# nico-bohlinger/RL-X

Hardware: AMD Instinct MI355X
Metric: env-steps/sec (whole node) PPO 4096 envs at 1/2/4/8 MI355X (higher is better)
Workload: dtype f32

## Files before the change

### include/rlx_hip.h

```cpp
#ifndef RLX_HIP_H
#define RLX_HIP_H

#include <stdint.h>

#ifdef __cplusplus
extern "C" {
#endif

#define RLX_OK 0
#define RLX_EINVAL (-1)
#define RLX_EHIP (-2)
#define RLX_ENOMEM (-3)
#define RLX_EUNSUP (-4)

#define RLX_ACT_TANH 0
#define RLX_ACT_ELU 1
#define RLX_ACT_RELU 2
#define RLX_ACT_NONE 3
#define RLX_ACT_SILU 4

#define RLX_THREEFRY_LEGACY 0
#define RLX_THREEFRY_PARTITIONABLE 1

typedef struct rlx_ctx rlx_ctx;
// ... 31 lines not shown
const char* rlx_prof_kernel_name(int k);
int rlx_prof_begin(rlx_ctx* ctx);
int rlx_prof_end(rlx_ctx* ctx, double* ms_out, double* flops_out, double* bytes_out, int64_t* count_out);
typedef struct rlx_prof_row {
  int32_t kernel;
  int32_t engine;
  int32_t N, K;
  int64_t M;
  int64_t launches, timed;
  double ms, flops, bytes;
} rlx_prof_row;
int rlx_prof_rows(rlx_ctx* ctx, rlx_prof_row* rows, int capacity, int* n_out);
int rlx_prof_union_ms(rlx_ctx* ctx, double* out);

int rlx_dbg_set_option(rlx_ctx* ctx, const char* name, int value);
int rlx_dbg_get_counter(rlx_ctx* ctx, const char* name, int64_t* out);

int rlx_dbg_set_sac_noise(rlx_ctx* ctx, const float* eps_next, const float* eps_cur);

int rlx_dbg_set_stamps(rlx_ctx* ctx, void* stamps);

int rlx_dbg_gemm_f32(rlx_ctx* ctx, int mode, const float* A, const float* B, float* C, float* aux, int64_t M, int N,
                     int K, int act, void* stream);

int rlx_dbg_l1_f32(rlx_ctx* ctx, int bwd, const float* X, const float* W, const float* b, const float* g,
                   const float* be, float* H, float* ln_partials, int64_t M, int O, int Hd, int act, int ln, int grid,
                   void* stream);

int rlx_threefry_split_host(const uint32_t key_in[2], uint32_t* keys_out , int num, int scheme);
int rlx_random_bits_u32(rlx_ctx*, const uint32_t key[2], uint32_t* out, int64_t n, int scheme, void* stream);
int rlx_normal_f32(rlx_ctx*, const uint32_t key[2], float* out, int64_t n, int scheme, void* stream);
int rlx_permutation_i32(rlx_ctx*, uint32_t key_io[2], int32_t* out, int E, int64_t B, int scheme, void* stream);

int rlx_env_reset_f32(rlx_ctx*, uint32_t seed, int env_id_offset, int N, int obs_dim, int horizon,
                      float* obs , int32_t* ep_step , float* ep_ret ,
                      float* last_ret , float* last_len , void* stream);
int rlx_env_step_f32(rlx_ctx*, uint32_t seed, int env_id_offset, uint32_t t, int N, int obs_dim, int act_dim,
                     int horizon, float p_term, float reward_noise,
                     const float* action , float* obs ,
                     float* final_obs ,
                     float* reward , float* terminated , float* truncated ,
                     int32_t* ep_step, float* ep_ret, float* last_ret, float* last_len,
                     float* episode_stats ,
                     void* stream);
int rlx_env_step_copy_f32(rlx_ctx*, uint32_t seed, int env_id_offset, uint32_t t, int N, int obs_dim, int act_dim,
                          int horizon, float p_term, float reward_noise, const float* action, float* obs, float* final_obs,
// ... 328 lines not shown
```

### rl-x_amd/csrc/common.h

```cpp
#pragma once
#include <hip/hip_runtime.h>
#include <hip/hip_ext.h>
#include <stdint.h>
#include <cstring>
#include <cmath>
#include <string>
#include <vector>
#include <functional>
#include "../../include/rlx_hip.h"

namespace rlx {

void set_error(const std::string& msg);

#define RLX_HIP_TRY(expr)                                                                      \
  do {                                                                                         \
    hipError_t e_ = (expr);                                                                    \
    if (e_ != hipSuccess) {                                                                    \
      ::rlx::set_error(std::string(#expr) + " failed: " + hipGetErrorString(e_) + " (" __FILE__ \
                       ":" + std::to_string(__LINE__) + ")");                                  \
      return RLX_EHIP;                                                                         \
    }                                                                                          \
  } while (0)

// ... 61 lines not shown
  int opt_flip = 0;
  hipStream_t side = nullptr;
  hipEvent_t ev_fork = nullptr, ev_join = nullptr;
  hipEvent_t ev_rows[2] = {nullptr, nullptr};
  hipEvent_t ev_cdone[2] = {nullptr, nullptr};
  const float* dbg_sac_eps[2] = {nullptr, nullptr};
  bool l1fwd_mfma = true;
  bool pipeline_updates = true;
  bool pf_valid = false;
  uint32_t pf_key_in[2] = {0, 0}, pf_key_out[2] = {0, 0};
  int pf_E = 0, pf_scheme = 0;
  int64_t pf_B = 0;
  hipEvent_t pf_done = nullptr;
  hipEvent_t ev_perm_free = nullptr;
  bool perm_free_recorded = false;
  bool two_streams = true;
  const uint32_t* l1_xmax = nullptr;
  const uint32_t* xmax_slot[2] = {nullptr, nullptr};
  int lf_idle_cus = 0;
  bool dw_recompute = false;
  float* l12_stats = nullptr;
  bool l12_ran = false;
  bool dw_merge = true;
  void* dbg_stamps = nullptr;
  bool fwd2h = true;
  int gather_group_rows = 524288;
  bool gather_records = true;
  bool l12_fused = true;
  int ppo_tail = -1;
  int ppo_twin = -1;
  bool fused_recurrent_act = true;
  int num_cus = 256;
  void* defer = nullptr;
  bool prof_on = false;
  int prof_sample = 1;
  hipEvent_t prof_ref = nullptr;
  double prof_union_ms = 0.0;
  std::vector<rlx::ProfRec> prof_recs;
  std::vector<rlx::ProfRow> prof_rows;
  std::vector<hipEvent_t> prof_pool;
  bool gemm_bx = true;
  float bx_gscale = 1.f;
  bool adam_emit = true;
  bool bx_keep[3] = {false, false, false};
  struct RoImages { bool valid = false; const float* params[2] = {nullptr, nullptr}; const void* img[2][3] = {}; int nt[2][3] = {}; } ro_img;
  int bx_force_mi = 0;
// ... 362 lines not shown
```

### rl-x_amd/csrc/core.hip

```cpp
#include "common.h"
#include <algorithm>
#include <cstdio>
#include <cstdlib>
#include <utility>

namespace rlx {

static thread_local std::string g_last_error;

void set_error(const std::string& msg) { g_last_error = msg; }

void* scratch(rlx_ctx* ctx, ScratchSlot s, size_t bytes) {
  Scratch& sl = ctx->slots[ctx->bank][s];
  if (sl.bytes >= bytes && sl.ptr) return sl.ptr;
  if (sl.ptr) {
    if (hipDeviceSynchronize() != hipSuccess) { set_error("hipDeviceSynchronize failed in scratch()"); return nullptr; }
    (void)hipFree(sl.ptr);
    sl.ptr = nullptr;
    sl.bytes = 0;
  }
  size_t want = ((bytes > (size_t(1) << 20) ? bytes + bytes / 8 : bytes) + 255) & ~size_t(255);
  void* p = nullptr;
  hipError_t e = hipMalloc(&p, want);
  if (e != hipSuccess) {
// ... 178 lines not shown
    rows[i] = rlx_prof_row{q.kid, q.engine, q.N, q.K, q.M, q.launches, q.timed, q.ms, q.flops, q.bytes};
  }
  return RLX_OK;
}

int rlx_prof_union_ms(rlx_ctx* ctx, double* out) {
  RLX_REQUIRE(ctx && out, RLX_EINVAL, "rlx_prof_union_ms: NULL pointer");
  *out = ctx->prof_union_ms;
  return RLX_OK;
}

int rlx_dbg_set_option(rlx_ctx* ctx, const char* name, int value) {
  RLX_REQUIRE(ctx && name, RLX_EINVAL, "rlx_dbg_set_option: NULL");
  if (std::string(name) == "sac_twin") { ctx->sac_twin = value; return RLX_OK; }
  if (std::string(name) == "disable_l1fused") { ctx->disable_l1fused = value != 0; return RLX_OK; }
  if (std::string(name) == "l1fwd_mfma") { ctx->l1fwd_mfma = value != 0; return RLX_OK; }
  if (std::string(name) == "pipeline_updates") { ctx->pipeline_updates = value != 0; return RLX_OK; }
  if (std::string(name) == "two_streams") { ctx->two_streams = value != 0; return RLX_OK; }
  if (std::string(name) == "ppo_twin") { ctx->ppo_twin = value; return RLX_OK; }
  if (std::string(name) == "ro_exit") { ctx->ro_exit = value; return RLX_OK; }
  if (std::string(name) == "lf_idle_cus") { ctx->lf_idle_cus = value < 0 ? 0 : value; return RLX_OK; }
  if (std::string(name) == "dw_recompute") { ctx->dw_recompute = value != 0; return RLX_OK; }
  if (std::string(name) == "dw_merge") { ctx->dw_merge = value != 0; return RLX_OK; }
  if (std::string(name) == "fwd2h") { ctx->fwd2h = value != 0; return RLX_OK; }
  if (std::string(name) == "l12_fused") { ctx->l12_fused = value != 0; return RLX_OK; }
  if (std::string(name) == "gather_group_rows") { ctx->gather_group_rows = value; return RLX_OK; }
  if (std::string(name) == "gather_records") { ctx->gather_records = value != 0; return RLX_OK; }
  if (std::string(name) == "ppo_tail") { ctx->ppo_tail = value < 0 ? -1 : (value > 2 ? 2 : value); return RLX_OK; }
  if (std::string(name) == "bx_force_mi") { ctx->bx_force_mi = value; return RLX_OK; }
  if (std::string(name) == "adam_emit") { ctx->adam_emit = value != 0; return RLX_OK; }
  if (std::string(name) == "bx_debug") { ctx->bx_debug = value; return RLX_OK; }
  if (std::string(name) == "bx_gscale_log2") { ctx->bx_gscale = ldexpf(1.f, value < 0 ? 0 : (value > 40 ? 40 : value)); return RLX_OK; }
  if (std::string(name) == "gemm_bx") { ctx->gemm_bx = value != 0; return RLX_OK; }
  if (std::string(name) == "prof_sample") { ctx->prof_sample = value < 1 ? 1 : value; return RLX_OK; }
  if (std::string(name) == "fused_recurrent_act") { ctx->fused_recurrent_act = value != 0; return RLX_OK; }
  RLX_REQUIRE(false, RLX_EINVAL, "rlx_dbg_set_option: unknown option");
}

int rlx_dbg_get_counter(rlx_ctx* ctx, const char* name, int64_t* out) {
  RLX_REQUIRE(ctx && name && out, RLX_EINVAL, "rlx_dbg_get_counter: NULL");
  int bank = 0, slot = 0;
  if (sscanf(name, "scratch_ptr:%d:%d", &bank, &slot) == 2 && bank >= 0 && bank < 3 && slot >= 0 && slot < rlx::SL_COUNT) {
    *out = (int64_t)reinterpret_cast<uintptr_t>(ctx->slots[bank][slot].ptr);
    return RLX_OK;
  }
  if (sscanf(name, "scratch_bytes:%d:%d", &bank, &slot) == 2 && bank >= 0 && bank < 3 && slot >= 0 && slot < rlx::SL_COUNT) {
    *out = (int64_t)ctx->slots[bank][slot].bytes;
    return RLX_OK;
  }
  if (std::string(name) == "allreduce_calls") { *out = ctx->ar_calls; return RLX_OK; }
  if (std::string(name) == "bx_window_fallbacks") { *out = ctx->bx_window_fallbacks; return RLX_OK; }
  if (std::string(name) == "gemm_bx") { *out = ctx->gemm_bx ? 1 : 0; return RLX_OK; }
  RLX_REQUIRE(false, RLX_EINVAL, "rlx_dbg_get_counter: unknown counter");
}

int rlx_version(void) { return 200; }

const char* rlx_last_error(void) { return rlx::g_last_error.c_str(); }

int rlx_ctx_create(int device, rlx_ctx** out) {
  RLX_REQUIRE(out != nullptr, RLX_EINVAL, "rlx_ctx_create: out is NULL");
  int count = 0;
  RLX_HIP_TRY(hipGetDeviceCount(&count));
  RLX_REQUIRE(device >= 0 && device < count, RLX_EINVAL, "rlx_ctx_create: no such HIP device");
  RLX_HIP_TRY(hipSetDevice(device));
  hipDeviceProp_t prop;
  RLX_HIP_TRY(hipGetDeviceProperties(&prop, device));
  rlx_ctx* c = new rlx_ctx();
  c->device = device;
  c->num_cus = prop.multiProcessorCount;
  if (const char* e = getenv("RLX_GEMM_BX")) c->gemm_bx = atoi(e) != 0;
  if (const char* e = getenv("RLX_BX_DEBUG")) c->bx_debug = atoi(e);
  *out = c;
  return RLX_OK;
}
// ... 42 lines not shown
```

### rl-x_amd/csrc/gemm_bx.hip

```cpp
#include "gemm_bx.h"
#ifndef RLX_WS_MIN_WAVES
#define RLX_WS_MIN_WAVES 2
#endif
#include "mlp.h"

namespace rlx {

__global__ __launch_bounds__(256) void k_bx_wfrag(BxJobs jobs) {
  int ji = 0;
#pragma unroll
  for (int q = 1; q < BX_MAX_JOBS; ++q)
    if (q < jobs.n && (int)blockIdx.x >= jobs.job[q].first_block) ji = q;
  const BxJob& jb = jobs.job[ji];
  const int idx = ((int)blockIdx.x - jb.first_block) * 256 + threadIdx.x;
  if (idx >= jb.KB * jb.NT * 64) return;
  const int lane = idx & 63, blk = idx >> 6, nt = blk % jb.NT, kb = blk / jb.NT;
  const int j = nt * 32 + (lane & 31), k0 = kb * 16 + 8 * (lane >> 5);
  float v[8];
#pragma unroll
  for (int e = 0; e < 8; ++e) {
    const int k = k0 + e;
    v[e] = (k < jb.K && j < jb.N) ? (jb.trans ? jb.W[(int64_t)j * jb.ldw + k] : jb.W[(int64_t)k * jb.ldw + j]) : 0.f;
  }
  u32x4 pl[X_NP];
// ... 146 lines not shown
    return;
  }
#pragma unroll
  for (int j = 0; j < 2; ++j) {
    const int col = n0 + acc_col(wn, j, lane);
    if (col >= N) continue;
#pragma unroll
    for (int i = 0; i < MI; ++i)
#pragma unroll
      for (int r = 0; r < 16; ++r) {
        const int64_t row = m0 + wm * 32 * MI + i * 32 + (r & 3) + 8 * (r >> 2) + 4 * (lane >> 5);
        if (row < M) {
          const int64_t o = row * ldc + col;
          float v = acc[i][j][r] * so;
          if (MODE == 0) v = act_fwd_t<ACT>(v + bv[j]);
          else if (APPLY) v *= act_grad_t<ACT>((Hsrc ? Hsrc : C)[o]);
          C[o] = v;
        }
      }
  }
}

constexpr int XW_THREADS = 512;
struct DwArgs {
  const float* Hp;
  const float* dZ;
  float* partW;
  float* partB;
  const float *Hp1, *dZ1;
  float *partW1, *partB1;
  int64_t M, Mc;
  int Kd, ldh, N, ntk, ntn;
  BxDwRecompute rc;
};
template <bool TWIN, bool REC = false>
__global__ __launch_bounds__(XW_THREADS, 2) void k_gemm_dw_bx(DwArgs a, DwArgs b, int nb0, float sg, float so) {
  extern __shared__ __attribute__((aligned(16))) char lds[];
  int bid = blockIdx.x, nblk = nb0;
  if (bid >= nb0) {
    a = b;
    bid -= nb0;
    nblk = gridDim.x - nb0;
  }
  const float* __restrict__ Hp = a.Hp;
  const float* __restrict__ dZ = a.dZ;
  float* __restrict__ partW = a.partW;
  float* __restrict__ partB = a.partB;
  if (TWIN && blockIdx.y) {
    Hp = a.Hp1;
    dZ = a.dZ1;
    partW = a.partW1;
    partB = a.partB1;
  }
  const int64_t M = a.M, Mc = a.Mc;
  const int Kd = a.Kd, ldh = a.ldh, N = a.N, ntk = a.ntk, ntn = a.ntn;
  const int ntiles = ntk * ntn;
  const int lb = xcd_remap(bid, nblk);
  const int s = lb / ntiles, tile = lb % ntiles;
  const int k0d = (tile / ntn) * G_BM;
  const int n0 = (tile % ntn) * G_BN;
  const int64_t mbeg = (int64_t)s * Mc;
  int64_t mend = mbeg + Mc;
  if (mend > M) mend = M;
  const int t = threadIdx.x, lane = t & 63, wv = t >> 6;
  const int nk = (int)((mend - mbeg + X_BK - 1) / X_BK);
  const bool interior = k0d + G_BM <= Kd && n0 + G_BN <= N;
  float colsum[4] = {0.f, 0.f, 0.f, 0.f};
  const int pt = t & 255, op = pt >> 7, tt = pt & 127, cg = tt & 31, mg = tt >> 5;
  const bool rec = REC && a.rc.X != nullptr;
  if (REC && wv >= 4 && rec && op == 0) {
    const BxDwRecompute& R = a.rc;
    const int wh = wv - 4, li = lane & 31, lh = lane >> 5;
    const int O = R.O;
    const int64_t pdelta = (TWIN && blockIdx.y) ? R.pdelta1 : 0;
    const float* __restrict__ stats = (TWIN && blockIdx.y) ? R.stats1 : R.stats;
    const u32x4* __restrict__ W1x = reinterpret_cast<const u32x4*>((TWIN && blockIdx.y) ? R.W1x1 : R.W1x);
    const float xs = R.xmax ? x_scale_from_max(*R.xmax, X_ASCALE) : X_ASCALE;
    const float xinv = 1.0f / xs;
    u32x4 w1f[2][2][X_NP];
    float bias[2], gam[2], bet[2];
#pragma unroll
    for (int j = 0; j < 2; ++j) {
      const int ctg = (k0d >> 5) + 2 * wh + j;
#pragma unroll
      for (int kb = 0; kb < 2; ++kb)
#pragma unroll
        for (int p = 0; p < X_NP; ++p) w1f[kb][j][p] = W1x[((int64_t)(kb * R.NT1 + ctg) * X_NP + p) * 64 + lane];
      const int col = k0d + 32 * (2 * wh + j) + li;
      bias[j] = R.b1[pdelta + col];
      gam[j] = R.g[pdelta + col];
      bet[j] = R.be[pdelta + col];
    }
    char* xa = lds + 4 * X_OPER + wh * (X_NP * 2048 + 256);
    float* st_l = reinterpret_cast<float*>(xa + X_NP * 2048);
    for (int i = lane; i < X_NP * 2048 / 16; i += 64) reinterpret_cast<u32x4*>(xa)[i] = u32x4{0u, 0u, 0u, 0u};
    constexpr int XC = 9;
    int xr_[XC], xk_[XC];
#pragma unroll
    for (int c = 0; c < XC; ++c) {
      const int e = lane + 64 * c;
      xr_[c] = e / O;
      xk_[c] = e - xr_[c] * O;
    }
    float xv[XC], smean = 0.f, srstd = 0.f;
    auto xload = [&](int kt) {
      const int64_t m0 = mbeg + (int64_t)kt * X_BK;
      const float* xb = R.X + m0 * O;
      const int nvalid = (int)((mend - m0 < X_BK ? mend - m0 : X_BK)) * O;
#pragma unroll
      for (int c = 0; c < XC; ++c) {
        const int e = lane + 64 * c;
        xv[c] = e < nvalid ? xb[e] : 0.f;
      }
      const bool rv = lane < 32 && m0 + lane < mend;
      smean = rv ? stats[m0 + lane] : 0.f;
      srstd = rv ? stats[M + m0 + lane] : 0.f;
// ... 53 lines not shown
    };
    xload(0);
    produce(0);
    if (nk > 1) xload(1);
    __syncthreads();
    for (int kt = 0; kt < nk; ++kt) {
      if (kt + 1 < nk) {
        produce((kt + 1) & 1);
        if (kt + 2 < nk) xload(kt + 2);
      }
      __syncthreads();
    }
    if (k0d == 0 && partB) {
      const float* red = reinterpret_cast<const float*>(lds);
      __syncthreads();
      if (pt < 128 && n0 + pt < N) partB[(int64_t)s * N + n0 + pt] = (red[pt] + red[128 + pt]) + (red[256 + pt] + red[384 + pt]);
    }
    return;
  }
  if (wv >= 4) {
    const float* __restrict__ src = op ? dZ : Hp;
    const int ld = op ? N : ldh, c0 = (op ? n0 : k0d) + cg * 4, ncols = op ? N : Kd;
    const bool plain = interior && (mend - mbeg) % X_BK == 0;
    float4 rra[8];
    const int rbase = rec ? 16 * (mg >> 1) + 4 * (mg & 1) : mg * 8;
    const float* sp = src + (mbeg + rbase) * ld + c0;
    auto load_plain = [&](int kt, float4 (&rr)[8]) {
      const int64_t m0 = (int64_t)kt * X_BK;
#pragma unroll
      for (int e = 0; e < 8; ++e) rr[e] = *reinterpret_cast<const float4*>(sp + (m0 + (rec ? (e & 3) + 8 * (e >> 2) : e)) * ld);
    };
    auto load_edge = [&](int kt, float4 (&rr)[8]) {
      const int64_t m0 = (int64_t)kt * X_BK;
#pragma unroll
      for (int e = 0; e < 8; ++e) rr[e] = ld4(src, mbeg + m0 + rbase + (rec ? (e & 3) + 8 * (e >> 2) : e), c0, mend, ncols, ld);
    };
    const float sc = op ? sg : X_ASCALE;
    auto stage = [&](int buf, const float4 (&rr)[8]) {
      char* dst = lds + buf * 2 * X_OPER + op * X_OPER;
      float v[8];
#pragma unroll
      for (int e = 0; e < 8; ++e) v[e] = rr[e].x;
      bx_stage_k8<true>(dst, cg * 4 + 0, mg, v, sc);
      if (op) {
#pragma unroll
        for (int e = 0; e < 8; ++e) colsum[0] += v[e];
      }
#pragma unroll
      for (int e = 0; e < 8; ++e) v[e] = rr[e].y;
      bx_stage_k8<true>(dst, cg * 4 + 1, mg, v, sc);
      if (op) {
#pragma unroll
        for (int e = 0; e < 8; ++e) colsum[1] += v[e];
      }
#pragma unroll
      for (int e = 0; e < 8; ++e) v[e] = rr[e].z;
      bx_stage_k8<true>(dst, cg * 4 + 2, mg, v, sc);
      if (op) {
#pragma unroll
        for (int e = 0; e < 8; ++e) colsum[2] += v[e];
      }
#pragma unroll
      for (int e = 0; e < 8; ++e) v[e] = rr[e].w;
      bx_stage_k8<true>(dst, cg * 4 + 3, mg, v, sc);
      if (op) {
#pragma unroll
        for (int e = 0; e < 8; ++e) colsum[3] += v[e];
      }
    };
    float4 rrb[8];
    auto clampk = [&](int kt) { return kt < nk ? kt : nk - 1; };
    auto produce = [&](auto load) {
      load(0, rra);
      load(clampk(1), rrb);
      stage(0, rra);
      load(clampk(2), rra);
      __syncthreads();
      int kt = 0;
      for (; kt + 2 <= nk; kt += 2) {
        if (kt + 1 < nk) stage((kt + 1) & 1, rrb);
        load(clampk(kt + 3), rrb);
        __syncthreads();
        if (kt + 2 < nk) stage((kt + 2) & 1, rra);
        load(clampk(kt + 4), rra);
        __syncthreads();
      }
      if (kt < nk) {
        __syncthreads();
      }
    };
    if (plain) produce(load_plain);
    else produce(load_edge);
    if (k0d == 0 && partB) {
      float* red = reinterpret_cast<float*>(lds);
      if (op) {
#pragma unroll
        for (int q = 0; q < 4; ++q) red[mg * 128 + cg * 4 + q] = colsum[q];
      }
      __syncthreads();
      if (pt < 128 && n0 + pt < N) partB[(int64_t)s * N + n0 + pt] = (red[pt] + red[128 + pt]) + (red[256 + pt] + red[384 + pt]);
    }
    return;
  }
  const int wm = wv >> 1, wn = wv & 1;
  f32x16 acc[2][2];
  zero_acc(acc);
  u32x4 fa[2][X_NP], fb[2][X_NP];
  __syncthreads();
  for (int kt = 0; kt < nk; ++kt) {
    const char* cur = lds + (kt & 1) * 2 * X_OPER;
    bx_load_frag<2, true>(cur, wm * 64, lane, 0, fa);
    bx_load_frag<2, true>(cur + X_OPER, wn * 64, lane, 0, fb);
    bx_mma<2>(fa, fb, acc);
    bx_load_frag<2, true>(cur, wm * 64, lane, 1, fa);
    bx_load_frag<2, true>(cur + X_OPER, wn * 64, lane, 1, fb);
    bx_mma<2>(fa, fb, acc);
    __syncthreads();
  }
  float* outW = partW + (int64_t)s * Kd * N;
  if (interior) {
    float* ob = outW + (int64_t)(k0d + wm * 64 + 4 * (lane >> 5)) * N + n0 + wn * 64 + (lane & 31);
#pragma unroll
    for (int i = 0; i < 2; ++i)
#pragma unroll
      for (int j = 0; j < 2; ++j)
#pragma unroll
        for (int r = 0; r < 16; ++r) ob[(i * 32 + (r & 3) + 8 * (r >> 2)) * N + j * 32] = acc[i][j][r] * so;
  } else {
#pragma unroll
    for (int j = 0; j < 2; ++j) {
      const int col = n0 + acc_col(wn, j, lane);
      if (col >= N) continue;
#pragma unroll
      for (int i = 0; i < 2; ++i)
#pragma unroll
        for (int r = 0; r < 16; ++r) {
          const int row = k0d + acc_row(wm, i, r, lane);
          if (row < Kd) outW[(int64_t)row * N + col] = acc[i][j][r] * so;
        }
    }
  }
  if (k0d == 0 && partB) __syncthreads();
}

static void add_job(BxJobs& jobs, int& blocks, int64_t& entries, const float* W, int ldw, int K, int N, int trans) {
  BxJob& j = jobs.job[jobs.n++];
  j.W = W;
  j.ldw = ldw;
  j.K = K;
  j.N = N;
  j.trans = trans;
  j.KB = 2 * div_up(K, X_BK);
  j.NT = 4 * div_up(N, G_BN);
  j.first_block = blocks;
  j.out = reinterpret_cast<u32x4*>(entries);
  blocks += div_up(j.KB * j.NT * 64, 256);
  entries += (int64_t)j.KB * j.NT * X_NP * 64;
}

int bx_prepare_mlp(rlx_ctx* ctx, const rlx_mlp_desc& d, const MlpLayout& L, const float* params, bool with_bwd,
                   hipStream_t st) {
  const int bank = ctx->bank;
  ctx->bx_n[bank] = 0;
  if (!ctx->gemm_bx) return RLX_OK;
  BxJobs jobs;
// ... 256 lines not shown
  const int ntn = div_up(Kd, G_BN);
  if (tw && bx_row_tiles(ctx, M, ntn) != 1) {
    RLX_BX_LAUNCH_WS_TWIN(1, act, apply, dim3(div_up(M, G_BM) * ntn, 2), st, dZ, (const u32x4*)img, (const float*)nullptr, HD, M, Kd,
                          N, N, ldo, ntn, (const int32_t*)nullptr, *tw, gs, X_WINV / gs, hsrc);
  } else if (tw) {
    RLX_BX_LAUNCH_TWIN(1, act, apply, dim3(div_up(M, 64) * ntn, 2), st, dZ, (const u32x4*)img, (const float*)nullptr, HD, M, Kd,
                       N, N, ldo, ntn, (const int32_t*)nullptr, *tw, gs, X_WINV / gs, hsrc);
  } else if (bx_row_tiles(ctx, M, ntn) == 1) {
    RLX_BX_LAUNCH_MI(1, 1, act, apply, dim3(div_up(M, 64) * ntn), st, dZ, (const u32x4*)img, (const float*)nullptr, HD, M, Kd, N,
                     N, ldo, ntn, (const int32_t*)nullptr, Twin{}, gs, X_WINV / gs, hsrc);
  } else {
    RLX_BX_LAUNCH_WS(1, act, apply, dim3(div_up(M, G_BM) * ntn), st, dZ, (const u32x4*)img, (const float*)nullptr, HD, M, Kd,
                     N, N, ldo, ntn, (const int32_t*)nullptr, Twin{}, gs, X_WINV / gs, hsrc);
  }
  RLX_LAUNCH_CHECK();
  return RLX_OK;
}

bool bx_dw_usable(const rlx_ctx* ctx, int64_t M, int Kd, int ldh, int N) {
  return !(ctx->bx_debug & 64) && ctx->gemm_bx && M >= 4096 && N % 4 == 0 && ldh % 4 == 0 && ldh >= ((Kd + 3) & ~3);
}

static int dw_attr() {
  static AttrOnce attr_set;      
  if (!attr_set.done()) {
    RLX_HIP_TRY(hipFuncSetAttribute(reinterpret_cast<const void*>(k_gemm_dw_bx<false>), hipFuncAttributeMaxDynamicSharedMemorySize,
                                    4 * X_OPER + 16384));
    RLX_HIP_TRY(hipFuncSetAttribute(reinterpret_cast<const void*>(k_gemm_dw_bx<true>), hipFuncAttributeMaxDynamicSharedMemorySize,
                                    4 * X_OPER + 16384));
    RLX_HIP_TRY(hipFuncSetAttribute(reinterpret_cast<const void*>(k_gemm_dw_bx<false, true>), hipFuncAttributeMaxDynamicSharedMemorySize,
                                    4 * X_OPER + 16384));
    RLX_HIP_TRY(hipFuncSetAttribute(reinterpret_cast<const void*>(k_gemm_dw_bx<true, true>), hipFuncAttributeMaxDynamicSharedMemorySize,
                                    4 * X_OPER + 16384));
    attr_set.mark();  
  }
  return RLX_OK;
}

static DwArgs dw_args(const float* Hp, const float* dZ, float* pW, float* pB, int64_t M, int Kd, int ldh, int N, int64_t Mc, int ntk,
                      int ntn, const Twin* tw) {
  DwArgs a;
  a.Hp = Hp; a.dZ = dZ; a.partW = pW; a.partB = pB;
  a.Hp1 = tw ? static_cast<const float*>(tw->p[0]) : nullptr;
  a.dZ1 = tw ? static_cast<const float*>(tw->p[1]) : nullptr;
  a.partW1 = tw ? const_cast<float*>(static_cast<const float*>(tw->p[2])) : nullptr;
  a.partB1 = tw ? const_cast<float*>(static_cast<const float*>(tw->p[3])) : nullptr;
  a.M = M; a.Mc = Mc; a.Kd = Kd; a.ldh = ldh; a.N = N; a.ntk = ntk; a.ntn = ntn;
  a.rc = BxDwRecompute{};
  return a;
}
constexpr size_t DW_REC_LDS = 2 * (X_NP * 2048 + 256);

int bx_launch_dw(rlx_ctx* ctx, const float* Hp, const float* dZ, float* pW, float* pB, int64_t M, int Kd, int ldh, int N,
                 int64_t Mc, int S, int ntk, int ntn, hipStream_t st, const Twin* tw) {
  int rc = dw_attr();
  if (rc) return rc;
  const float gs = ctx->bx_gscale;
  ProfScope prof(ctx, PK_GEMM_DW, (tw ? 4.0 : 2.0) * (double)M * Kd * N, st, (tw ? 2.0 : 1.0) * gemm_bytes(Kd, N, M), Kd, N, (int)M, 1);
  const DwArgs a = dw_args(Hp, dZ, pW, pB, M, Kd, ldh, N, Mc, ntk, ntn, tw);
  const int nb = S * ntk * ntn;
  if (tw) {
    RLX_PLAUNCH(k_gemm_dw_bx<true>, dim3(nb, 2), dim3(XW_THREADS), 4 * X_OPER, st, a, a, nb, gs, X_AINV / gs);
  } else {
    RLX_PLAUNCH(k_gemm_dw_bx<false>, dim3(nb), dim3(XW_THREADS), 4 * X_OPER, st, a, a, nb, gs, X_AINV / gs);
  }
  RLX_LAUNCH_CHECK();
  return RLX_OK;
}

int bx_launch_dw2(rlx_ctx* ctx, const BxDwJob& j0, const BxDwJob& j1, int64_t M, hipStream_t st, const Twin* tw0, const Twin* tw1) {
  int rc = dw_attr();
  if (rc) return rc;
  RLX_REQUIRE((tw0 == nullptr) == (tw1 == nullptr), RLX_EINVAL, "bx_launch_dw2: both jobs or neither must have a twin");
  const float gs = ctx->bx_gscale;
  const double nets = tw0 ? 2.0 : 1.0;
  ProfScope prof(ctx, PK_GEMM_DW, nets * 2.0 * (double)M * ((double)j0.Kd * j0.N + (double)j1.Kd * j1.N), st,
                 nets * (gemm_bytes(j0.Kd, j0.N, M) + gemm_bytes(j1.Kd, j1.N, M)), j0.Kd + j1.Kd, j0.N + j1.N, (int)M, 1);
  DwArgs a = dw_args(j0.Hp, j0.dZ, j0.pW, j0.pB, M, j0.Kd, j0.ldh, j0.N, j0.Mc, j0.ntk, j0.ntn, tw0);
  const DwArgs b = dw_args(j1.Hp, j1.dZ, j1.pW, j1.pB, M, j1.Kd, j1.ldh, j1.N, j1.Mc, j1.ntk, j1.ntn, tw1);
  if (j0.rc) {
    RLX_REQUIRE(j0.rc->X && j0.rc->W1x && j0.rc->stats && j0.Kd == 512 && j0.rc->O <= 32 && (!tw0 || (j0.rc->W1x1 && j0.rc->stats1)),
                RLX_EINVAL, "bx_launch_dw2: incomplete recompute description");
    a.rc = *j0.rc;
  }
  const int nb0 = j0.S * j0.ntk * j0.ntn, nb1 = j1.S * j1.ntk * j1.ntn;
  const size_t lds = 4 * X_OPER + (j0.rc ? DW_REC_LDS : 0);
  if (j0.rc) {
    if (tw0) { RLX_PLAUNCH((k_gemm_dw_bx<true, true>), dim3(nb0 + nb1, 2), dim3(XW_THREADS), lds, st, a, b, nb0, gs, X_AINV / gs); }
    else { RLX_PLAUNCH((k_gemm_dw_bx<false, true>), dim3(nb0 + nb1), dim3(XW_THREADS), lds, st, a, b, nb0, gs, X_AINV / gs); }
  } else if (tw0) {
    RLX_PLAUNCH(k_gemm_dw_bx<true>, dim3(nb0 + nb1, 2), dim3(XW_THREADS), lds, st, a, b, nb0, gs, X_AINV / gs);
  } else {
    RLX_PLAUNCH(k_gemm_dw_bx<false>, dim3(nb0 + nb1), dim3(XW_THREADS), lds, st, a, b, nb0, gs, X_AINV / gs);
  }
  RLX_LAUNCH_CHECK();
  return RLX_OK;
}

}
```

### rl-x_amd/csrc/mlp.hip

```cpp
#include "mlp.h"
#include "ln_kernels.h"

namespace rlx {

constexpr int L1_R_FWD = 4, L1_R_BWD = 2;
constexpr int L1_MAXJ = 8;
constexpr int L1_THREADS = 512;

__device__ __forceinline__ float readlane_f(float v, int lane) {
  return __int_as_float(__builtin_amdgcn_readlane(__float_as_int(v), lane));
}

struct L1Args {
  const float* X;
  float* H;
  int64_t M;
  int O, Hd, NJ;
};

template <bool BWD, int ACT, bool LN, int L1R>
__device__ __forceinline__ void l1_rows(const L1Args& a, const float* __restrict__ Ws, const float* __restrict__ bs,
                                        const float* __restrict__ gs, const float* __restrict__ bes,
                                        float (&dg)[L1_MAXJ], float (&dbe)[L1_MAXJ], int lane, int64_t wave_g,
                                        int64_t nwaves) {
// ... 1502 lines not shown
    o.W = 0;
    o.in = K;
    o.out = N;
    const bool was = ctx->gemm_bx;
    ctx->gemm_bx = true;
    int rc = bx_prepare_mlp(ctx, d, L, B, mode == 4, st);
    if (!rc) {
      if (mode == 3) {
        RLX_REQUIRE(aux, RLX_EINVAL, "rlx_dbg_gemm_f32: mode 3 needs bias");
        const void* img = bx_lookup(ctx, B, 0, K, N);
        rc = img ? bx_launch_fwd(ctx, A, img, aux, C, M, N, K, act, st, 0, nullptr) : RLX_EUNSUP;
      } else {
        const void* img = bx_lookup(ctx, B, 1, N, K);
        rc = img ? bx_launch_dx(ctx, A, img, C, M, N, K, K, act >= 0 ? act : 0, act >= 0 ? 1 : 0, st) : RLX_EUNSUP;
      }
    }
    bx_release(ctx);
    ctx->gemm_bx = was;
    return rc;
  }
  RLX_REQUIRE(false, RLX_EINVAL, "rlx_dbg_gemm_f32: mode must be 0 .. 5");
}

extern "C" int rlx_dbg_l1_f32(rlx_ctx* ctx, int bwd, const float* X, const float* W, const float* b, const float* g,
                              const float* be, float* H, float* ln_partials, int64_t M, int O, int Hd, int act, int ln,
                              int grid, void* stream) {
  RLX_REQUIRE(ctx && X && W && b && H && M > 0 && O >= 1 && O <= 32 && Hd % 64 == 0 && Hd <= 512 && grid > 0,
              RLX_EINVAL, "rlx_dbg_l1_f32: bad args");
  if (bwd) return launch_l1<true>(X, W, b, g, be, H, ln_partials, M, O, Hd, act, ln, grid, (hipStream_t)stream);
  return launch_l1<false>(X, W, b, g, be, H, nullptr, M, O, Hd, act, ln, grid, (hipStream_t)stream);
}

extern "C" int rlx_mlp_fwd_f32(rlx_ctx* ctx, const rlx_mlp_desc* desc, const float* params, const float* x, float* out,
                               int64_t n, void* stream) {
  RLX_REQUIRE(ctx && desc && params && x && out && n >= 0, RLX_EINVAL, "rlx_mlp_fwd_f32: bad args");
  if (n == 0) return RLX_OK;
  int rc = mlp_check_desc(*desc);
  if (rc) return rc;
  const MlpLayout L = make_layout(*desc);
  hipStream_t st = (hipStream_t)stream;
  int maxh = 0;
  for (int l = 0; l < desc->n_hidden; ++l) maxh = desc->hidden[l] > maxh ? desc->hidden[l] : maxh;
  float* bufA = (float*)scratch(ctx, SL_FWD_A, (size_t)n * maxh * sizeof(float));
  float* bufB = (float*)scratch(ctx, SL_FWD_B, (size_t)n * maxh * sizeof(float));
  if (!bufA || !bufB) return RLX_ENOMEM;
  float* acts[4] = {bufA, bufB, bufA, bufB};
// ... 30 lines not shown
```

### rl-x_amd/rlx_amd/hip/lib.py

```python
import ctypes
import os
from ctypes import POINTER, Structure, c_char_p, c_float, c_int, c_int32, c_int64, c_uint32, c_void_p

import numpy as np

ACT_TANH, ACT_ELU, ACT_RELU = 0, 1, 2
THREEFRY_LEGACY, THREEFRY_PARTITIONABLE = 0, 1

_PKG_ROOT = os.path.dirname(os.path.dirname(os.path.dirname(os.path.abspath(__file__))))


def library_path():
    return os.environ.get("RLX_HIP_LIBRARY", os.path.join(_PKG_ROOT, "lib", "librlxhip.so"))


class RlxError(RuntimeError):
    pass


class MlpDesc(Structure):
    _fields_ = [("in_dim", c_int32), ("n_hidden", c_int32), ("hidden", c_int32 * 4), ("out_dim", c_int32),
                ("act", c_int32), ("ln_first", c_int32), ("has_logstd", c_int32)]


# ... 111 lines not shown
class ProfRow(ctypes.Structure):
    _fields_ = [("kernel", ctypes.c_int32), ("engine", ctypes.c_int32), ("N", ctypes.c_int32), ("K", ctypes.c_int32),
                ("M", c_int64), ("launches", c_int64), ("timed", c_int64), ("ms", ctypes.c_double),
                ("flops", ctypes.c_double), ("bytes", ctypes.c_double)]


_ALLREDUCE_FN = ctypes.CFUNCTYPE(c_int, c_void_p, c_void_p, c_int64, c_int, c_int)
_U32P = POINTER(c_uint32)
_I64P = POINTER(c_int64)
_DESCP = POINTER(MlpDesc)
_HPP = POINTER(PpoHparams)
_F32HP = POINTER(c_float)
_SACHPP = POINTER(SacHparams)
_LDESCP = POINTER(LstmPolicyDesc)

_SIGNATURES = {
    "rlx_version": (c_int, []),
    "rlx_last_error": (c_char_p, []),
    "rlx_ctx_create": (c_int, [c_int, POINTER(c_void_p)]),
    "rlx_ctx_destroy": (c_int, [c_void_p]),
    "rlx_mlp_param_count": (c_int64, [_DESCP]),
    "rlx_dbg_gemm_f32": (c_int, [c_void_p, c_int, c_void_p, c_void_p, c_void_p, c_void_p, c_int64, c_int, c_int, c_int,
                                 c_void_p]),
    "rlx_dbg_l1_f32": (c_int, [c_void_p, c_int] + [c_void_p] * 7 + [c_int64, c_int, c_int, c_int, c_int, c_int, c_void_p]),
    "rlx_dbg_set_option": (c_int, [c_void_p, c_char_p, c_int]),
    "rlx_dbg_get_counter": (c_int, [c_void_p, c_char_p, _I64P]),
    "rlx_dbg_set_sac_noise": (c_int, [c_void_p, c_void_p, c_void_p]),
    "rlx_dbg_set_stamps": (c_int, [c_void_p, c_void_p]),
    "rlx_dist_rccl_path": (c_char_p, []),
    "rlx_c51_critic_loss_f32": (c_int, [c_void_p] * 11 + [c_int64, c_int, c_float, c_float, c_float, c_int, c_void_p, c_void_p, c_void_p, c_void_p]),
    "rlx_obs_norm_update_f32": (c_int, [c_void_p, c_void_p, c_int64, c_int, c_void_p, c_void_p, c_void_p, c_void_p, c_void_p]),
    "rlx_obs_norm_apply_f32": (c_int, [c_void_p, c_void_p, c_int64, c_int, c_void_p, c_void_p, c_float, c_void_p, c_void_p]),
    "rlx_prof_begin": (c_int, [c_void_p]),
    "rlx_prof_union_ms": (c_int, [c_void_p, POINTER(ctypes.c_double)]),
    "rlx_prof_kernel_count": (c_int, []),
    "rlx_prof_kernel_name": (c_char_p, [c_int]),
    "rlx_prof_end": (c_int, [c_void_p, POINTER(ctypes.c_double), POINTER(ctypes.c_double), POINTER(ctypes.c_double), _I64P]),
    "rlx_prof_rows": (c_int, [c_void_p, c_void_p, c_int, POINTER(c_int)]),
    "rlx_threefry_split_host": (c_int, [_U32P, _U32P, c_int, c_int]),
    "rlx_random_bits_u32": (c_int, [c_void_p, _U32P, c_void_p, c_int64, c_int, c_void_p]),
    "rlx_normal_f32": (c_int, [c_void_p, _U32P, c_void_p, c_int64, c_int, c_void_p]),
    "rlx_permutation_i32": (c_int, [c_void_p, _U32P, c_void_p, c_int, c_int64, c_int, c_void_p]),
    "rlx_env_reset_f32": (c_int, [c_void_p, c_uint32, c_int, c_int, c_int, c_int] + [c_void_p] * 5 + [c_void_p]),
    "rlx_env_step_f32": (c_int, [c_void_p, c_uint32, c_int, c_uint32, c_int, c_int, c_int, c_int, c_float, c_float]
                         + [c_void_p] * 11 + [c_void_p]),
    "rlx_env_step_copy_f32": (c_int, [c_void_p, c_uint32, c_int, c_uint32, c_int, c_int, c_int, c_int, c_float, c_float]
# ... 252 lines not shown
        _check(self.lib.rlx_prof_union_ms(self.h, ctypes.byref(out)), "rlx_prof_union_ms")
        return out.value

    def set_option(self, name, value):
        _check(self.lib.rlx_dbg_set_option(self.h, name.encode(), int(value)), "rlx_dbg_set_option")

    def get_counter(self, name):
        out = c_int64()
        _check(self.lib.rlx_dbg_get_counter(self.h, name.encode(), ctypes.byref(out)), "rlx_dbg_get_counter")
        return out.value

    def dbg_set_sac_noise(self, eps_next=None, eps_cur=None):
        f = self.torch.float32
        _check(self.lib.rlx_dbg_set_sac_noise(self.h, _ptr(eps_next, f, True), _ptr(eps_cur, f, True)), "rlx_dbg_set_sac_noise")

    def dbg_set_stamps(self, stamps=None):
        _check(self.lib.rlx_dbg_set_stamps(self.h, c_void_p(stamps.data_ptr()) if stamps is not None else None), "rlx_dbg_set_stamps")

    def dbg_gemm(self, mode, A, B, C, aux, M, N, K, act):
        f = self.torch.float32
        _check(self.lib.rlx_dbg_gemm_f32(self.h, mode, _ptr(A, f), _ptr(B, f), _ptr(C, f), _ptr(aux, f, True), M, N, K,
                                         act, _stream()), "rlx_dbg_gemm_f32")

    def dbg_l1(self, bwd, X, W, b, g, be, H, ln_partials, act, ln, grid):
        f = self.torch.float32
        M, O = X.shape
        _check(self.lib.rlx_dbg_l1_f32(self.h, int(bwd), _ptr(X, f), _ptr(W, f), _ptr(b, f), _ptr(g, f, True),
                                       _ptr(be, f, True), _ptr(H, f), _ptr(ln_partials, f, True), M, O, H.shape[1],
                                       act, int(ln), grid, _stream()), "rlx_dbg_l1_f32")

    def random_bits(self, key, out, scheme=THREEFRY_PARTITIONABLE):
        t = self.torch
        _check(self.lib.rlx_random_bits_u32(self.h, _key_arr(key), _ptr(out, t.int32), out.numel(), scheme, _stream()),
               "rlx_random_bits_u32")

    def normal(self, key, out, scheme=THREEFRY_PARTITIONABLE):
        t = self.torch
        _check(self.lib.rlx_normal_f32(self.h, _key_arr(key), _ptr(out, t.float32), out.numel(), scheme, _stream()),
               "rlx_normal_f32")

    def permutation(self, key, out, E, B, scheme=THREEFRY_PARTITIONABLE):
        t = self.torch
        k = _key_arr(key)
        if out.numel() != E * B:
            raise RlxError("permutation: out must hold E*B int32")
        _check(self.lib.rlx_permutation_i32(self.h, k, _ptr(out, t.int32), E, B, scheme, _stream()),
# ... 569 lines not shown
```

Before: 7.617 million.

## Deepen weight-gradient GEMM load/stage ring to 3-4 buffers when grid fits CUs

Generalizes the dW GEMM producer loop from a fixed double buffer to a templated ring of depth D (2-4) of register prefetches and LDS slots. A new kernel variant with launch bounds of one block per CU and larger LDS is used when the workgroup count fits within the CU count. The goal is to hide global-load latency better when occupancy is low, at the cost of more registers and LDS per block. Also adds a debug entry point, an option and counter for the ring depth, and compile-time stamp instrumentation.

```diff
diff --git a/include/rlx_hip.h b/include/rlx_hip.h
--- a/include/rlx_hip.h
+++ b/include/rlx_hip.h
@@ -77,6 +77,9 @@
 
 int rlx_dbg_gemm_f32(rlx_ctx* ctx, int mode, const float* A, const float* B, float* C, float* aux, int64_t M, int N,
                      int K, int act, void* stream);
+
+int rlx_dbg_dw_slabs_f32(rlx_ctx* ctx, const float* Hp0, const float* dZ0, int K0, int N0, const float* Hp1, const float* dZ1,
+                         int K1, int N1, int64_t M, int64_t Mc, float* out, void* stream);
 
 int rlx_dbg_l1_f32(rlx_ctx* ctx, int bwd, const float* X, const float* W, const float* b, const float* g,
                    const float* be, float* H, float* ln_partials, int64_t M, int O, int Hd, int act, int ln, int grid,
diff --git a/rl-x_amd/csrc/common.h b/rl-x_amd/csrc/common.h
--- a/rl-x_amd/csrc/common.h
+++ b/rl-x_amd/csrc/common.h
@@ -107,6 +107,8 @@
   float* l12_stats = nullptr;
   bool l12_ran = false;
   bool dw_merge = true;
+  int dw_ring = 0;
+  int dw_ring_last = 0;
   void* dbg_stamps = nullptr;
   bool fwd2h = true;
   int gather_group_rows = 524288;
diff --git a/rl-x_amd/csrc/core.hip b/rl-x_amd/csrc/core.hip
--- a/rl-x_amd/csrc/core.hip
+++ b/rl-x_amd/csrc/core.hip
@@ -224,6 +224,11 @@
   if (std::string(name) == "lf_idle_cus") { ctx->lf_idle_cus = value < 0 ? 0 : value; return RLX_OK; }
   if (std::string(name) == "dw_recompute") { ctx->dw_recompute = value != 0; return RLX_OK; }
   if (std::string(name) == "dw_merge") { ctx->dw_merge = value != 0; return RLX_OK; }
+  if (std::string(name) == "dw_ring") {
+    RLX_REQUIRE(value == 0 || (value >= 2 && value <= 4), RLX_EINVAL, "rlx_dbg_set_option: dw_ring is 0 (automatic), 2, 3 or 4");
+    ctx->dw_ring = value;
+    return RLX_OK;
+  }
   if (std::string(name) == "fwd2h") { ctx->fwd2h = value != 0; return RLX_OK; }
   if (std::string(name) == "l12_fused") { ctx->l12_fused = value != 0; return RLX_OK; }
   if (std::string(name) == "gather_group_rows") { ctx->gather_group_rows = value; return RLX_OK; }
@@ -253,6 +258,7 @@
   if (std::string(name) == "allreduce_calls") { *out = ctx->ar_calls; return RLX_OK; }
   if (std::string(name) == "bx_window_fallbacks") { *out = ctx->bx_window_fallbacks; return RLX_OK; }
   if (std::string(name) == "gemm_bx") { *out = ctx->gemm_bx ? 1 : 0; return RLX_OK; }
+  if (std::string(name) == "dw_ring") { *out = ctx->dw_ring_last; return RLX_OK; }
   RLX_REQUIRE(false, RLX_EINVAL, "rlx_dbg_get_counter: unknown counter");
 }
 
diff --git a/rl-x_amd/csrc/gemm_bx.hip b/rl-x_amd/csrc/gemm_bx.hip
--- a/rl-x_amd/csrc/gemm_bx.hip
+++ b/rl-x_amd/csrc/gemm_bx.hip
@@ -192,6 +192,9 @@
 }
 
 constexpr int XW_THREADS = 512;
+#ifndef RLX_DW_STAMPS
+#define RLX_DW_STAMPS 0
+#endif
 struct DwArgs {
   const float* Hp;
   const float* dZ;
@@ -202,9 +205,13 @@
   int64_t M, Mc;
   int Kd, ldh, N, ntk, ntn;
   BxDwRecompute rc;
+#if RLX_DW_STAMPS
+  unsigned long long* stamps;
+#endif
 };
-template <bool TWIN, bool REC = false>
-__global__ __launch_bounds__(XW_THREADS, 2) void k_gemm_dw_bx(DwArgs a, DwArgs b, int nb0, float sg, float so) {
+template <bool TWIN, bool REC, int D>
+__device__ __forceinline__ void gemm_dw_bx_body(DwArgs a, const DwArgs& b, int nb0, float sg, float so) {
+  static_assert(D >= 2 && D <= 4 && (!REC || D == 2), "ring depth");
   extern __shared__ __attribute__((aligned(16))) char lds[];
   int bid = blockIdx.x, nblk = nb0;
   if (bid >= nb0) {
@@ -238,6 +245,25 @@
   float colsum[4] = {0.f, 0.f, 0.f, 0.f};
   const int pt = t & 255, op = pt >> 7, tt = pt & 127, cg = tt & 31, mg = tt >> 5;
   const bool rec = REC && a.rc.X != nullptr;
+#if RLX_DW_STAMPS
+  unsigned long long* const stp = (blockIdx.x == 0 && blockIdx.y == 0 && lane == 0 && (wv == 0 || wv == 4)) ? a.stamps : nullptr;
+  const long long st_t0 = clock64(), st_w0 = wall_clock64();
+  long long st_last = st_t0, st_wait = 0, st_work = 0, st_bar = 0;
+#define DW_TICK(ACC) { const long long c_ = clock64(); ACC += c_ - st_last; st_last = c_; }
+#define DW_WAIT(RR) { DW_TICK(st_work) asm volatile("" :: "v"(RR[7].x), "v"(RR[7].y), "v"(RR[7].z), "v"(RR[7].w)); DW_TICK(st_wait) }
+#define DW_WORK_END() DW_TICK(st_work)
+#define DW_BARRIER() { DW_TICK(st_work) __syncthreads(); DW_TICK(st_bar) }
+#define DW_FINISH(BASE)                                                                   \
+  if (stp) {                                                                              \
+    stp[(BASE) + 0] = clock64() - st_t0; stp[(BASE) + 1] = st_wait; stp[(BASE) + 2] = st_work; \
+    stp[(BASE) + 3] = st_bar; stp[(BASE) + 4] = nk; stp[(BASE) + 5] = wall_clock64() - st_w0;  \
+  }
+#else
+#define DW_WAIT(RR)
+#define DW_WORK_END()
+#define DW_BARRIER() __syncthreads();
+#define DW_FINISH(BASE)
+#endif
   if (REC && wv >= 4 && rec && op == 0) {
     const BxDwRecompute& R = a.rc;
     const int wh = wv - 4, li = lane & 31, lh = lane >> 5;
@@ -261,7 +287,7 @@
       gam[j] = R.g[pdelta + col];
       bet[j] = R.be[pdelta + col];
     }
-    char* xa = lds + 4 * X_OPER + wh * (X_NP * 2048 + 256);
+    char* xa = lds + 2 * D * X_OPER + wh * (X_NP * 2048 + 256);
     float* st_l = reinterpret_cast<float*>(xa + X_NP * 2048);
     for (int i = lane; i < X_NP * 2048 / 16; i += 64) reinterpret_cast<u32x4*>(xa)[i] = u32x4{0u, 0u, 0u, 0u};
     constexpr int XC = 9;
@@ -361,7 +387,6 @@
     const float* __restrict__ src = op ? dZ : Hp;
     const int ld = op ? N : ldh, c0 = (op ? n0 : k0d) + cg * 4, ncols = op ? N : Kd;
     const bool plain = interior && (mend - mbeg) % X_BK == 0;
-    float4 rra[8];
     const int rbase = rec ? 16 * (mg >> 1) + 4 * (mg & 1) : mg * 8;
     const float* sp = src + (mbeg + rbase) * ld + c0;
     auto load_plain = [&](int kt, float4 (&rr)[8]) {
@@ -407,29 +432,37 @@
         for (int e = 0; e < 8; ++e) colsum[3] += v[e];
       }
     };
-    float4 rrb[8];
+    float4 rr[D][8];
     auto clampk = [&](int kt) { return kt < nk ? kt : nk - 1; };
     auto produce = [&](auto load) {
-      load(0, rra);
-      load(clampk(1), rrb);
-      stage(0, rra);
-      load(clampk(2), rra);
-      __syncthreads();
+#pragma unroll
+      for (int d = 0; d < D; ++d) load(clampk(d), rr[d]);
+      DW_WAIT(rr[0])
+      stage(0, rr[0]);
+      load(clampk(D), rr[0]);
+      DW_BARRIER()
       int kt = 0;
-      for (; kt + 2 <= nk; kt += 2) {
-        if (kt + 1 < nk) stage((kt + 1) & 1, rrb);
-        load(clampk(kt + 3), rrb);
-        __syncthreads();
-        if (kt + 2 < nk) stage((kt + 2) & 1, rra);
-        load(clampk(kt + 4), rra);
-        __syncthreads();
-      }
-      if (kt < nk) {
-        __syncthreads();
+      for (; kt + D <= nk; kt += D) {
+#pragma unroll
+        for (int d = 1; d <= D; ++d) {
+          DW_WAIT(rr[d % D])
+          if (kt + d < nk) stage(d % D, rr[d % D]);
+          load(clampk(kt + d + D), rr[d % D]);
+          DW_BARRIER()
+        }
+      }
+#pragma unroll
+      for (int d = 1; d < D; ++d) {
+        if (kt + d <= nk) {
+          DW_WAIT(rr[d])
+          if (d < D - 1 && kt + d < nk) stage(d, rr[d]);
+          DW_BARRIER()
+        }
       }
     };
     if (plain) produce(load_plain);
     else produce(load_edge);
+    DW_FINISH(0)
     if (k0d == 0 && partB) {
       float* red = reinterpret_cast<float*>(lds);
       if (op) {
@@ -445,17 +478,19 @@
   f32x16 acc[2][2];
   zero_acc(acc);
   u32x4 fa[2][X_NP], fb[2][X_NP];
-  __syncthreads();
-  for (int kt = 0; kt < nk; ++kt) {
-    const char* cur = lds + (kt & 1) * 2 * X_OPER;
+  DW_BARRIER()
+  for (int kt = 0, sl = 0; kt < nk; ++kt, sl = sl + 1 == D ? 0 : sl + 1) {
+    const char* cur = lds + sl * 2 * X_OPER;
     bx_load_frag<2, true>(cur, wm * 64, lane, 0, fa);
     bx_load_frag<2, true>(cur + X_OPER, wn * 64, lane, 0, fb);
     bx_mma<2>(fa, fb, acc);
     bx_load_frag<2, true>(cur, wm * 64, lane, 1, fa);
     bx_load_frag<2, true>(cur + X_OPER, wn * 64, lane, 1, fb);
     bx_mma<2>(fa, fb, acc);
-    __syncthreads();
-  }
+    DW_WORK_END()
+    DW_BARRIER()
+  }
+  DW_FINISH(8)
   float* outW = partW + (int64_t)s * Kd * N;
   if (interior) {
     float* ob = outW + (int64_t)(k0d + wm * 64 + 4 * (lane >> 5)) * N + n0 + wn * 64 + (lane & 31);
@@ -480,6 +515,20 @@
     }
   }
   if (k0d == 0 && partB) __syncthreads();
+#undef DW_TICK
+#undef DW_WAIT
+#undef DW_WORK_END
+#undef DW_BARRIER
+#undef DW_FINISH
+}
+
+template <bool TWIN, bool REC = false>
+__global__ __launch_bounds__(XW_THREADS, 2) void k_gemm_dw_bx(DwArgs a, DwArgs b, int nb0, float sg, float so) {
+  gemm_dw_bx_body<TWIN, REC, 2>(a, b, nb0, sg, so);
+}
+template <bool TWIN, int D>
+__global__ __launch_bounds__(XW_THREADS, 1) void k_gemm_dwring_bx(DwArgs a, DwArgs b, int nb0, float sg, float so) {
+  gemm_dw_bx_body<TWIN, false, D>(a, b, nb0, sg, so);
 }
 
 static void add_job(BxJobs& jobs, int& blocks, int64_t& entries, const float* W, int ldw, int K, int N, int trans) {
@@ -782,20 +831,32 @@
 }
 
 static int dw_attr() {
-  static AttrOnce attr_set;      
+  static AttrOnce attr_set;
   if (!attr_set.done()) {
-    RLX_HIP_TRY(hipFuncSetAttribute(reinterpret_cast<const void*>(k_gemm_dw_bx<false>), hipFuncAttributeMaxDynamicSharedMemorySize,
-                                    4 * X_OPER + 16384));
-    RLX_HIP_TRY(hipFuncSetAttribute(reinterpret_cast<const void*>(k_gemm_dw_bx<true>), hipFuncAttributeMaxDynamicSharedMemorySize,
-                                    4 * X_OPER + 16384));
-    RLX_HIP_TRY(hipFuncSetAttribute(reinterpret_cast<const void*>(k_gemm_dw_bx<false, true>), hipFuncAttributeMaxDynamicSharedMemorySize,
-                                    4 * X_OPER + 16384));
-    RLX_HIP_TRY(hipFuncSetAttribute(reinterpret_cast<const void*>(k_gemm_dw_bx<true, true>), hipFuncAttributeMaxDynamicSharedMemorySize,
-                                    4 * X_OPER + 16384));
-    attr_set.mark();  
+    const void* k2[4] = {reinterpret_cast<const void*>(k_gemm_dw_bx<false>), reinterpret_cast<const void*>(k_gemm_dw_bx<true>),
+                         reinterpret_cast<const void*>(k_gemm_dw_bx<false, true>), reinterpret_cast<const void*>(k_gemm_dw_bx<true, true>)};
+    for (const void* k : k2) RLX_HIP_TRY(hipFuncSetAttribute(k, hipFuncAttributeMaxDynamicSharedMemorySize, 4 * X_OPER + 16384));
+    RLX_HIP_TRY(hipFuncSetAttribute(reinterpret_cast<const void*>(k_gemm_dwring_bx<false, 3>), hipFuncAttributeMaxDynamicSharedMemorySize, 6 * X_OPER));
+    RLX_HIP_TRY(hipFuncSetAttribute(reinterpret_cast<const void*>(k_gemm_dwring_bx<true, 3>), hipFuncAttributeMaxDynamicSharedMemorySize, 6 * X_OPER));
+    RLX_HIP_TRY(hipFuncSetAttribute(reinterpret_cast<const void*>(k_gemm_dwring_bx<false, 4>), hipFuncAttributeMaxDynamicSharedMemorySize, 8 * X_OPER));
+    RLX_HIP_TRY(hipFuncSetAttribute(reinterpret_cast<const void*>(k_gemm_dwring_bx<true, 4>), hipFuncAttributeMaxDynamicSharedMemorySize, 8 * X_OPER));
+    attr_set.mark();
   }
   return RLX_OK;
 }
+
+static int dw_ring(rlx_ctx* ctx, int wgs, bool rec) {
+  int D = 2;
+  if (!rec) D = ctx->dw_ring ? ctx->dw_ring : (wgs <= ctx->num_cus ? 4 : 2);
+  ctx->dw_ring_last = D;
+  return D;
+}
+#define RLX_DW_LAUNCH(TWINV, DV, GRID, ST, ...)                                                                                    \
+  switch (DV) {                                                                                                                    \
+    case 4: RLX_PLAUNCH((k_gemm_dwring_bx<TWINV, 4>), GRID, dim3(XW_THREADS), 8 * X_OPER, ST, __VA_ARGS__); break;              \
+    case 3: RLX_PLAUNCH((k_gemm_dwring_bx<TWINV, 3>), GRID, dim3(XW_THREADS), 6 * X_OPER, ST, __VA_ARGS__); break;              \
+    default: RLX_PLAUNCH((k_gemm_dw_bx<TWINV>), GRID, dim3(XW_THREADS), 4 * X_OPER, ST, __VA_ARGS__); break;             \
+  }
 
 static DwArgs dw_args(const float* Hp, const float* dZ, float* pW, float* pB, int64_t M, int Kd, int ldh, int N, int64_t Mc, int ntk,
                       int ntn, const Twin* tw) {
@@ -817,12 +878,16 @@
   if (rc) return rc;
   const float gs = ctx->bx_gscale;
   ProfScope prof(ctx, PK_GEMM_DW, (tw ? 4.0 : 2.0) * (double)M * Kd * N, st, (tw ? 2.0 : 1.0) * gemm_bytes(Kd, N, M), Kd, N, (int)M, 1);
-  const DwArgs a = dw_args(Hp, dZ, pW, pB, M, Kd, ldh, N, Mc, ntk, ntn, tw);
+  DwArgs a = dw_args(Hp, dZ, pW, pB, M, Kd, ldh, N, Mc, ntk, ntn, tw);
+#if RLX_DW_STAMPS
+  a.stamps = (unsigned long long*)ctx->dbg_stamps;
+#endif
   const int nb = S * ntk * ntn;
+  const int D = dw_ring(ctx, nb * (tw ? 2 : 1), false);
   if (tw) {
-    RLX_PLAUNCH(k_gemm_dw_bx<true>, dim3(nb, 2), dim3(XW_THREADS), 4 * X_OPER, st, a, a, nb, gs, X_AINV / gs);
+    RLX_DW_LAUNCH(true, D, dim3(nb, 2), st, a, a, nb, gs, X_AINV / gs);
   } else {
-    RLX_PLAUNCH(k_gemm_dw_bx<false>, dim3(nb), dim3(XW_THREADS), 4 * X_OPER, st, a, a, nb, gs, X_AINV / gs);
+    RLX_DW_LAUNCH(false, D, dim3(nb), st, a, a, nb, gs, X_AINV / gs);
   }
   RLX_LAUNCH_CHECK();
   return RLX_OK;
@@ -843,15 +908,19 @@
                 RLX_EINVAL, "bx_launch_dw2: incomplete recompute description");
     a.rc = *j0.rc;
   }
+#if RLX_DW_STAMPS
+  a.stamps = (unsigned long long*)ctx->dbg_stamps;
+#endif
   const int nb0 = j0.S * j0.ntk * j0.ntn, nb1 = j1.S * j1.ntk * j1.ntn;
   const size_t lds = 4 * X_OPER + (j0.rc ? DW_REC_LDS : 0);
+  const int D = dw_ring(ctx, (nb0 + nb1) * (tw0 ? 2 : 1), j0.rc != nullptr);
   if (j0.rc) {
     if (tw0) { RLX_PLAUNCH((k_gemm_dw_bx<true, true>), dim3(nb0 + nb1, 2), dim3(XW_THREADS), lds, st, a, b, nb0, gs, X_AINV / gs); }
     else { RLX_PLAUNCH((k_gemm_dw_bx<false, true>), dim3(nb0 + nb1), dim3(XW_THREADS), lds, st, a, b, nb0, gs, X_AINV / gs); }
   } else if (tw0) {
-    RLX_PLAUNCH(k_gemm_dw_bx<true>, dim3(nb0 + nb1, 2), dim3(XW_THREADS), lds, st, a, b, nb0, gs, X_AINV / gs);
+    RLX_DW_LAUNCH(true, D, dim3(nb0 + nb1, 2), st, a, b, nb0, gs, X_AINV / gs);
   } else {
-    RLX_PLAUNCH(k_gemm_dw_bx<false>, dim3(nb0 + nb1), dim3(XW_THREADS), lds, st, a, b, nb0, gs, X_AINV / gs);
+    RLX_DW_LAUNCH(false, D, dim3(nb0 + nb1), st, a, b, nb0, gs, X_AINV / gs);
   }
   RLX_LAUNCH_CHECK();
   return RLX_OK;
diff --git a/rl-x_amd/csrc/mlp.hip b/rl-x_amd/csrc/mlp.hip
--- a/rl-x_amd/csrc/mlp.hip
+++ b/rl-x_amd/csrc/mlp.hip
@@ -1548,6 +1548,19 @@
   RLX_REQUIRE(false, RLX_EINVAL, "rlx_dbg_gemm_f32: mode must be 0 .. 5");
 }
 
+extern "C" int rlx_dbg_dw_slabs_f32(rlx_ctx* ctx, const float* Hp0, const float* dZ0, int K0, int N0, const float* Hp1,
+                                    const float* dZ1, int K1, int N1, int64_t M, int64_t Mc, float* out, void* stream) {
+  RLX_REQUIRE(ctx && Hp0 && dZ0 && out && M > 0 && Mc > 0 && K0 > 0 && N0 > 0, RLX_EINVAL, "rlx_dbg_dw_slabs_f32: bad args");
+  RLX_REQUIRE((Hp1 != nullptr) == (dZ1 != nullptr) && (!Hp1 || (K1 > 0 && N1 > 0)), RLX_EINVAL, "rlx_dbg_dw_slabs_f32: incomplete second job");
+  RLX_REQUIRE(K0 % 4 == 0 && N0 % 4 == 0 && (!Hp1 || (K1 % 4 == 0 && N1 % 4 == 0)), RLX_EUNSUP, "rlx_dbg_dw_slabs_f32: N and K must be multiples of 4");
+  const int S = (int)div_up(M, Mc);
+  BxDwJob j0{Hp0, dZ0, out, out + (size_t)S * K0 * N0, K0, K0, N0, Mc, S, div_up(K0, G_BM), div_up(N0, G_BN)};
+  if (!Hp1) return bx_launch_dw(ctx, Hp0, dZ0, j0.pW, j0.pB, M, K0, K0, N0, Mc, S, j0.ntk, j0.ntn, (hipStream_t)stream);
+  float* o1 = j0.pB + (size_t)S * N0;
+  BxDwJob j1{Hp1, dZ1, o1, o1 + (size_t)S * K1 * N1, K1, K1, N1, Mc, S, div_up(K1, G_BM), div_up(N1, G_BN)};
+  return bx_launch_dw2(ctx, j0, j1, M, (hipStream_t)stream);
+}
+
 extern "C" int rlx_dbg_l1_f32(rlx_ctx* ctx, int bwd, const float* X, const float* W, const float* b, const float* g,
                               const float* be, float* H, float* ln_partials, int64_t M, int O, int Hd, int act, int ln,
                               int grid, void* stream) {
diff --git a/rl-x_amd/rlx_amd/hip/lib.py b/rl-x_amd/rlx_amd/hip/lib.py
--- a/rl-x_amd/rlx_amd/hip/lib.py
+++ b/rl-x_amd/rlx_amd/hip/lib.py
@@ -157,6 +157,8 @@
     "rlx_mlp_param_count": (c_int64, [_DESCP]),
     "rlx_dbg_gemm_f32": (c_int, [c_void_p, c_int, c_void_p, c_void_p, c_void_p, c_void_p, c_int64, c_int, c_int, c_int,
                                  c_void_p]),
+    "rlx_dbg_dw_slabs_f32": (c_int, [c_void_p, c_void_p, c_void_p, c_int, c_int, c_void_p, c_void_p, c_int, c_int, c_int64, c_int64,
+                                     c_void_p, c_void_p]),
     "rlx_dbg_l1_f32": (c_int, [c_void_p, c_int] + [c_void_p] * 7 + [c_int64, c_int, c_int, c_int, c_int, c_int, c_void_p]),
     "rlx_dbg_set_option": (c_int, [c_void_p, c_char_p, c_int]),
     "rlx_dbg_get_counter": (c_int, [c_void_p, c_char_p, _I64P]),
@@ -455,6 +457,13 @@
         _check(self.lib.rlx_dbg_gemm_f32(self.h, mode, _ptr(A, f), _ptr(B, f), _ptr(C, f), _ptr(aux, f, True), M, N, K,
                                          act, _stream()), "rlx_dbg_gemm_f32")
 
+    def dbg_dw_slabs(self, Hp0, dZ0, Mc, out, Hp1=None, dZ1=None):
+        f = self.torch.float32
+        M, K0 = Hp0.shape
+        K1, N1 = (Hp1.shape[1], dZ1.shape[1]) if Hp1 is not None else (0, 0)
+        _check(self.lib.rlx_dbg_dw_slabs_f32(self.h, _ptr(Hp0, f), _ptr(dZ0, f), K0, dZ0.shape[1], _ptr(Hp1, f, True), _ptr(dZ1, f, True),
+                                             K1, N1, M, int(Mc), _ptr(out, f), _stream()), "rlx_dbg_dw_slabs_f32")
+
     def dbg_l1(self, bwd, X, W, b, g, be, H, ln_partials, act, ln, grid):
         f = self.torch.float32
         M, O = X.shape
```

After: 7.318 million. 0.961x the previous value.
